# lordnn/OF_DIS

Measured on AMD Instinct MI355X. Metric: MPix/s (and frames/sec) 1080p op-point-2; avg EPE vs CPU ref, higher is better.
Workload: dtype f32; 1 GPU; run_OF_INT 1920x1080 op-point 2, 4096 pairs/GPU/step; width=1920, height=1080, channels=1, oppoint=2, batch_per_gpu=4096, streams=2, pairs_per_launch=2048, parallelism=frame-sharded x1

## Files before the change

### of_dis_amd/csrc/ofdis_internal.h

```cpp
#pragma once

#include <hip/hip_runtime.h>
#include <stdint.h>

namespace ofdis {

struct LevelGeom {
  int w, h;
  int pad;
  int W, H;
  int nopw, noph, npatch, offw, offh;
  float tmp_lb, tmp_ubw, tmp_ubh;
  int level;
};

struct PyrBaseArgs {
  const uint8_t *img_a, *img_b;
  int n, nf, W0, H0, noc;
  int padl, padt;
  int log2s;
  int w, h;
  float *out;
  int rgb_sad;
  int stereo;
};

struct PyrGradmagArgs {
  const uint8_t *img_a, *img_b;
  int n, nf, W0, H0, padl, padt, Wp, Hp;
  float *out;
  int stereo;
};

struct PyrDownArgs {
  const float *src;
  float *dst;
  int n2, w, h, noc;
};

struct PyrPadGradArgs {
  const float *lvl;
  float *img, *dx, *dy;
  int n2, w, h, noc, pad;
  int per_value;
};

struct PatchArgs {
  const float *img_a, *dx_a, *dy_a, *img_b;
  const float *prev;
  long prev_frame_stride;
  int prev_comp_stride, prev_elem_stride, prev_w;
  float *p_iter;
  float *pweight;
  int n, nop, noc, p, novals, steps;
  int costfct, patnorm, max_iter, min_iter;
  float dp_thresh_sq, dr_thresh, res_thresh, outlierthresh;
  float outlier_sq;
  int camlr;
  int wave_per_patch;
  int generic;
  int window;
  int quad;
  int x16;
  int absw;
  int aslots;
  int buf32;
  int fdiv;
  int maxres;
  int stage;
  LevelGeom g;
};

struct AggArgs {
  const float *p_iter, *pweight;
  const float *cg_p_iter, *cg_pweight;
  float *flow;
  int n, nop, noc, p, novals, steps;
  int absw;
  int aslots;
  int stage;
  LevelGeom g;
};

struct TvArgs {
  const float *img_a, *img_b;
  float *flow;
  float *wxs, *wys;
  float *du, *dv, *mask, *s;
  float *coef;
  float *t, *dt;
  float *Ix, *Iy, *Iz, *Ixx, *Ixy, *Iyy, *Ixz, *Iyz;
  long sp;
  int wrap;
  int skew_slots;
  int n, nop, noc, w, h, pad, W;
  float quarter_alpha, hdo3, hgo3, omega;
  int first_iter;
  int solverit;
  int camlr;
  int sor_generic;
  int sor_variant;
  int sor_point;
  int sor_cring;
  int sor_pack;
  int sor_rows2;
  int smsys;
  int prepd;
  int smsys2d;
  int smsys_prefetch;
  int smsys_small;
  int smsys_march;
  int smsys_deriv;
  int prepd_df;
  int sor_redblack;
  int lat;
};

struct UpArgs {
  const float *flow;
  float *out;
  int n, nop, wl, hl, log2s, W0, H0, offx, offy;
  int nt_store;
  int form;
  int f16, planar;
  float *out_r;
  int n_l;
};

struct LevelOutArgs {
  const float *flow;
  void *out;
  int n, nop, wl, hl, log2s;
  int f16, planar;
};

struct InitArgs {
  const float *init;
  float *out;
  int n, nop, W0, H0, padl, padt, log2k, wo, ho;
  float sc, scale;
};

struct FbArgs {
  const float *fw, *bw;
  uint8_t *occ_fw, *occ_bw;
  float *err_fw, *err_bw;
  int n, W, H;
  float alpha, beta;
};

struct FbLevelArgs {
  const float *gfw, *gbw;
  uint8_t *occ_fw, *occ_bw;
  float *err_fw, *err_bw;
  int n, W, H;
  float alpha, beta;
  int gw, gh, log2c, offx, offy;
};

struct LrArgs {
  const float *dl, *dr;
  uint8_t *occ_l, *occ_r;
  float *err_l, *err_r;
  int n, W, H;
  float alpha, beta;
};

struct WarpArgs {
  const uint8_t *img;
  const void *flow;
  void *out;
  uint8_t *valid;
  int n, W, H, noc;
  float scale;
  int out_f32;
  int f16, planar, level;
  int gw, gh, log2c, offx, offy;
};

constexpr int kInterpMaxT = 16;
struct InterpArgs {
  const uint8_t *img_a, *img_b;
  const void *flow_fw, *flow_bw;
  const uint8_t *occ_a, *occ_b;
  void *out;
  uint8_t *valid;
  int n, W, H, noc;
  int out_f32;
  int f16, planar, level;
  int gw, gh, log2c, offx, offy;
  int srows, scols;
  int nt;
  float t[kInterpMaxT];
};

void launch_warp(const WarpArgs &a, hipStream_t s);
// ... 32 lines not shown
```

### of_dis_amd/csrc/ofdis_kernels.hip

```cpp
#include "ofdis_internal.h"
#include "ofdis_math.h"

#include <algorithm>
#include <cstdlib>
#include <type_traits>
#include <utility>

#pragma clang fp contract(off)

namespace ofdis {
typedef float float4_u __attribute__((ext_vector_type(4), aligned(4)));
typedef float float4_v __attribute__((ext_vector_type(4)));

namespace {

#include "ofdis_tv_dev.inc"
#include "ofdis_agg_dev.inc"

inline unsigned ceil_div(long a, long b) { return (unsigned)((a + b - 1) / b); }

template <int V>
using Int = std::integral_constant<int, V>;
template <int... Vs, class F>
inline bool pick(int v, F &&f) {
// ... 98 lines not shown
          const uint4 v = reinterpret_cast<const uint4 *>(row)[q];
          s2 = __builtin_amdgcn_sad_u8(v.x, 0u, s2);
          s2 = __builtin_amdgcn_sad_u8(v.y, 0u, s2);
          s2 = __builtin_amdgcn_sad_u8(v.z, 0u, s2);
          s2 = __builtin_amdgcn_sad_u8(v.w, 0u, s2);
        }
      } else if (VB == 8) {
        const uint2 v = *reinterpret_cast<const uint2 *>(row);
        s2 = __builtin_amdgcn_sad_u8(v.x, 0u, s2);
        s2 = __builtin_amdgcn_sad_u8(v.y, 0u, s2);
      } else {
        s2 = __builtin_amdgcn_sad_u8(*reinterpret_cast<const unsigned *>(row), 0u, s2);
      }
      acc[by] = s2;
    }
#pragma unroll
    for (int by = 0; by < B; ++by) sum += acc[by];
  } else {
    for (int by = 0; by < B; ++by) {
      const int yy = clampi(y * B + by - a.padt, 0, a.H0 - 1);
      const uint8_t *row = src + (long)yy * a.W0;
      for (int bx = 0; bx < B; ++bx) {
        const int xc = clampi(x0 + bx, 0, a.W0 - 1);
        sum += row[ST && mir ? a.W0 - 1 - xc : xc];
      }
    }
  }
  a.out[t] = (float)sum * scale;
}

template <int L, bool ST = false>
__global__ __launch_bounds__(256) void k_pyr_base_rgb(PyrBaseArgs a) {
  constexpr int B = 1 << L, ND = 3 * B / 4;
  const long t = (long)blockIdx.x * 256 + threadIdx.x;
  if (t >= (long)a.nf * a.h * a.w) return;
  const int x = (int)(t % a.w);
  const long r = t / a.w;
  const int y = (int)(r % a.h), f = (int)(r / a.h);
  const long fs = (long)a.H0 * a.W0 * 3;
  bool mir;
  const uint8_t *src = pyr_src<ST>(a, f, fs, mir);
  const float scale = 1.0f / (float)(1 << (2 * L));
  const int x0 = x * B - a.padl;
  const int xs = ST && mir ? a.W0 - x0 - B : x0;
  unsigned sum[3] = {0u, 0u, 0u};
  if (x0 >= 0 && x0 + B <= a.W0 && (((uintptr_t)src + 3 * (long)xs) & 3) == 0 && ((3 * a.W0) & 3) == 0) {
    constexpr unsigned M[3][3] = {{0xFF0000FFu, 0x00FF0000u, 0x0000FF00u},
                                  {0x0000FF00u, 0xFF0000FFu, 0x00FF0000u},
                                  {0x00FF0000u, 0x0000FF00u, 0xFF0000FFu}};
    unsigned v[B][ND];
#pragma unroll
    for (int by = 0; by < B; ++by) {
      const int yy = clampi(y * B + by - a.padt, 0, a.H0 - 1);
      const unsigned *row = reinterpret_cast<const unsigned *>(src + ((long)yy * a.W0 + xs) * 3);
#pragma unroll
      for (int k = 0; k < ND; ++k) v[by][k] = row[k];
    }
#pragma unroll
    for (int by = 0; by < B; ++by)
#pragma unroll
      for (int k = 0; k < ND; ++k)
#pragma unroll
        for (int c = 0; c < 3; ++c) sum[c] = __builtin_amdgcn_sad_u8(v[by][k] & M[c][k % 3], 0u, sum[c]);
  } else {
    for (int c = 0; c < 3; ++c)
      for (int by = 0; by < B; ++by) {
        const int yy = clampi(y * B + by - a.padt, 0, a.H0 - 1);
        const uint8_t *row = src + (long)yy * a.W0 * 3 + c;
        for (int bx = 0; bx < B; ++bx) {
          const int xc = clampi(x0 + bx, 0, a.W0 - 1);
          sum[c] += row[(ST && mir ? a.W0 - 1 - xc : xc) * 3];
        }
      }
  }
#pragma unroll
  for (int c = 0; c < 3; ++c) a.out[t * 3 + c] = (float)sum[c] * scale;
}

__global__ __launch_bounds__(256) void k_pyr_down(PyrDownArgs a) {
  const int rw = a.w * a.noc;
  const long total = (long)a.n2 * a.h * rw;
  for (long t = (long)blockIdx.x * blockDim.x + threadIdx.x; t < total; t += (long)gridDim.x * blockDim.x) {
  const long r = t / rw;
  const int xc = (int)(t - r * rw), y = (int)(r % a.h), f = (int)(r / a.h);
  const int x = xc / a.noc, c = xc - x * a.noc;
  const long idx = (((long)f * a.h + y) * a.w + x) * a.noc + c;
  const int sw = 2 * a.w;
  const float *s = a.src + (long)f * (2 * a.h) * sw * a.noc;
  const float p = s[((2 * y) * sw + 2 * x) * a.noc + c], q = s[((2 * y) * sw + 2 * x + 1) * a.noc + c];
  const float u = s[((2 * y + 1) * sw + 2 * x) * a.noc + c], v = s[((2 * y + 1) * sw + 2 * x + 1) * a.noc + c];
  a.dst[idx] = ((p + q) + (u + v)) * 0.25f;
  }
}

__device__ __forceinline__ int reflect101(int i, int n) {
  if (n == 1) return 0;
  if (i < 0) return -i;
  if (i >= n) return 2 * n - 2 - i;
  return i;
}

template <bool ST = false>
__global__ __launch_bounds__(256) void k_pyr_gradmag(PyrGradmagArgs a) {
  const int X = blockIdx.x * blockDim.x + threadIdx.x, Y = blockIdx.y, f = blockIdx.z;
  if (X >= a.Wp) return;
  const long fs = (long)a.H0 * a.W0;
  bool mir = false;
  const uint8_t *src;
  if constexpr (ST) {
    const int q = f / a.n, i = f - q * a.n;
    mir = (q & 1) != 0;
    src = (q == 0 || q == 3 ? a.img_a : a.img_b) + (long)i * fs;
  } else {
    src = f < a.n ? a.img_a + (long)f * fs : a.img_b + (long)(f - a.n) * fs;
  }
  const int xm = reflect101(X - 1, a.Wp), xp = reflect101(X + 1, a.Wp);
  const int ym = reflect101(Y - 1, a.Hp), yp = reflect101(Y + 1, a.Hp);
  auto px = [&](int xx, int yy) {
    const int xc = clampi(xx - a.padl, 0, a.W0 - 1);
    return (float)src[(long)clampi(yy - a.padt, 0, a.H0 - 1) * a.W0 + (ST && mir ? a.W0 - 1 - xc : xc)];
  };
  const float tm = px(xp, ym) - px(xm, ym);
  const float t0 = px(xp, Y) - px(xm, Y);
  const float tp = px(xp, yp) - px(xm, yp);
  const float sm = (px(xm, ym) + px(xp, ym)) * 0.125f + px(X, ym) * 0.25f;
  const float sp = (px(xm, yp) + px(xp, yp)) * 0.125f + px(X, yp) * 0.25f;
  const float dx = (tm + tp) * 0.125f + t0 * 0.25f, dy = sp - sm;
  a.out[((long)f * a.Hp + Y) * a.Wp + X] = sqrtf(dx * dx + dy * dy);
}

__global__ __launch_bounds__(256) void k_pyr_pad_grad(PyrPadGradArgs a) {
  const int W = a.w + 2 * a.pad, H = a.h + 2 * a.pad;
  const long total = (long)a.n2 * H * W;
  for (long t = (long)blockIdx.x * blockDim.x + threadIdx.x; t < total; t += (long)gridDim.x * blockDim.x) {
  const long r = t / W;
  const int X = (int)(t - r * W), Y = (int)(r % H), f = (int)(r / H);
  const long idx = ((long)f * H + Y) * W + X;
  const int sx = X - a.pad, sy = Y - a.pad;
  const int noc = a.noc, w = a.w;
  const float *L = a.lvl + (long)f * a.h * a.w * noc;
  const bool inside = sx >= 0 && sx < a.w && sy >= 0 && sy < a.h;
  for (int c = 0; c < noc; ++c) {
    const long o = idx * noc + c;
    if (inside) {
      const int xm = reflect101(sx - 1, a.w), xp = reflect101(sx + 1, a.w);
      const int ym = reflect101(sy - 1, a.h), yp = reflect101(sy + 1, a.h);
#define PX(xx, yy) L[((yy) * w + (xx)) * noc + c]
      const float tm = PX(xp, ym) - PX(xm, ym);
      const float t0 = PX(xp, sy) - PX(xm, sy);
      const float tp = PX(xp, yp) - PX(xm, yp);
      const float sm = (PX(xm, ym) + PX(xp, ym)) * 0.125f + PX(sx, ym) * 0.25f;
      const float sp = (PX(xm, yp) + PX(xp, yp)) * 0.125f + PX(sx, yp) * 0.25f;
      a.img[o] = PX(sx, sy);
      a.dx[o] = (tm + tp) * 0.125f + t0 * 0.25f;
      a.dy[o] = sp - sm;
#undef PX
    } else {
      a.img[o] = L[(clampi(sy, 0, a.h - 1) * w + clampi(sx, 0, a.w - 1)) * noc + c];
      a.dx[o] = 0.0f;
      a.dy[o] = 0.0f;
    }
  }
  }
}

template <int NOC>
__global__ __launch_bounds__(256) void k_pyr_pad_grad_v(PyrPadGradArgs a) {
  const int W = a.w + 2 * a.pad, H = a.h + 2 * a.pad, RW = W * NOC;
  const long total = (long)a.n2 * H * RW;
  for (long t = (long)blockIdx.x * blockDim.x + threadIdx.x; t < total; t += (long)gridDim.x * blockDim.x) {
    const long r = t / RW;
    const int xc = (int)(t - r * RW), Y = (int)(r % H), f = (int)(r / H);
    const int X = xc / NOC, c = xc - X * NOC;
    const int sx = X - a.pad, sy = Y - a.pad;
    const int w = a.w;
    const float *L = a.lvl + (long)f * a.h * a.w * NOC;
    if (sx >= 0 && sx < a.w && sy >= 0 && sy < a.h) {
      const int xm = reflect101(sx - 1, a.w), xp = reflect101(sx + 1, a.w);
      const int ym = reflect101(sy - 1, a.h), yp = reflect101(sy + 1, a.h);
#define PX(xx, yy) L[((yy) * w + (xx)) * NOC + c]
      const float tm = PX(xp, ym) - PX(xm, ym);
      const float t0 = PX(xp, sy) - PX(xm, sy);
      const float tp = PX(xp, yp) - PX(xm, yp);
      const float sm = (PX(xm, ym) + PX(xp, ym)) * 0.125f + PX(sx, ym) * 0.25f;
      const float sp = (PX(xm, yp) + PX(xp, yp)) * 0.125f + PX(sx, yp) * 0.25f;
      a.img[t] = PX(sx, sy);
      a.dx[t] = (tm + tp) * 0.125f + t0 * 0.25f;
      a.dy[t] = sp - sm;
#undef PX
    } else {
      a.img[t] = L[(clampi(sy, 0, a.h - 1) * w + clampi(sx, 0, a.w - 1)) * NOC + c];
      a.dx[t] = 0.0f;
      a.dy[t] = 0.0f;
    }
  }
}

}
void launch_pyr_base(const PyrBaseArgs &a, hipStream_t s) {
  const unsigned blocks = ceil_div((long)a.nf * a.h * a.w, 256);
  if (a.stereo) {
    if (a.noc == 1 && pick<2, 3, 4, 5>(a.log2s, [&](auto L) { k_pyr_base_gray<L, true><<<blocks, 256, 0, s>>>(a); })) return;
    if (a.noc == 3 && a.rgb_sad && pick<2, 3, 4>(a.log2s, [&](auto L) { k_pyr_base_rgb<L, true><<<blocks, 256, 0, s>>>(a); }))
      return;
    k_pyr_base<true><<<dim3(ceil_div(a.w, 256), a.h, a.nf), 256, 0, s>>>(a);
    return;
  }
  if (a.noc == 1 && pick<2, 3, 4, 5>(a.log2s, [&](auto L) { k_pyr_base_gray<L><<<blocks, 256, 0, s>>>(a); })) return;
  if (a.noc == 3 && a.rgb_sad && pick<2, 3, 4>(a.log2s, [&](auto L) { k_pyr_base_rgb<L><<<blocks, 256, 0, s>>>(a); }))
    return;
  k_pyr_base<<<dim3(ceil_div(a.w, 256), a.h, a.nf), 256, 0, s>>>(a);
}
void launch_pyr_gradmag(const PyrGradmagArgs &a, hipStream_t s) {
  if (a.stereo) k_pyr_gradmag<true><<<dim3(ceil_div(a.Wp, 256), a.Hp, a.nf), 256, 0, s>>>(a);
  else k_pyr_gradmag<<<dim3(ceil_div(a.Wp, 256), a.Hp, a.nf), 256, 0, s>>>(a);
}
void launch_pyr_down(const PyrDownArgs &a, hipStream_t s) {
  k_pyr_down<<<std::min(ceil_div((long)a.n2 * a.h * a.w * a.noc, 256), 1u << 22), 256, 0, s>>>(a);
}
void launch_pyr_pad_grad(const PyrPadGradArgs &a, hipStream_t s) {
  const long px = (long)a.n2 * (a.h + 2 * a.pad) * (a.w + 2 * a.pad);
  if (a.noc == 3 && a.per_value) k_pyr_pad_grad_v<3><<<std::min(ceil_div(px * 3, 256), 1u << 22), 256, 0, s>>>(a);
  else k_pyr_pad_grad<<<std::min(ceil_div(px, 256), 1u << 22), 256, 0, s>>>(a);
}
namespace {


constexpr int kPatchWaves = 4;

template <int N>
__device__ __forceinline__ float row_shl(float v) {
  return __builtin_bit_cast(float, __builtin_amdgcn_update_dpp(0, __builtin_bit_cast(int, v), 0x100 + N, 0xF, 0xF, false));
}

template <int R, int JM>
__device__ __forceinline__ void eigen_reduce(const float *lds, int rs, int n, int lane, float (&out)[R]) {
  __builtin_amdgcn_fence(__ATOMIC_RELEASE, "wavefront");
  __builtin_amdgcn_wave_barrier();
  __builtin_amdgcn_fence(__ATOMIC_ACQUIRE, "wavefront");
  const int r = lane >> 3, s = lane & 7;
  const int pairs = n >> 3;
  const bool odd = ((n >> 2) & 1) != 0;
  float acc = 0.0f, first = 0.0f, tail = 0.0f;
  if (r < R) {
    if (JM == 1) {
      const float4 A = *reinterpret_cast<const float4 *>(lds + r * 64 + s * 8);
      const float4 B = *reinterpret_cast<const float4 *>(lds + r * 64 + s * 8 + 4);
      const float e[8] = {A.x, A.y, A.z, A.w, B.x, B.y, B.z, B.w};
      first = e[0];
      acc = first;
#pragma unroll
      for (int c = 1; c < 8; ++c)
        if (c < pairs) acc = acc + e[c];
#pragma unroll
      for (int c = 0; c < 8; ++c)
        if (c == pairs) tail = e[c];
    } else {
      const float *x = lds + r * rs;
      first = x[s];
      acc = first;
      for (int c = 1; c < pairs; ++c) acc = acc + x[s + 8 * c];
      tail = x[pairs * 8 + s];
    }
  }
  float rl = pairs > 0 ? acc + row_shl<4>(acc) : first;
  if (odd && pairs > 0) rl = rl + tail;
  const float t = rl + row_shl<2>(rl);
  const float tot = t + row_shl<1>(t);
#pragma unroll
  for (int k = 0; k < R; ++k)
    out[k] = __builtin_bit_cast(float, __builtin_amdgcn_readlane(__builtin_bit_cast(int, tot), k * 8));
  __builtin_amdgcn_wave_barrier();
}

template <int JM>
__device__ __forceinline__ void lds_store(float *lds, int n, int lane, const float (&v)[JM]) {
  if (JM == 1) {
    lds[(lane & 7) * 8 + (lane >> 3)] = lane < n ? v[0] : 0.0f;
    return;
  }
#pragma unroll
  for (int j = 0; j < JM; ++j) {
    const int e = lane + 64 * j;
    if (e < n) lds[e] = v[j];
  }
}

struct Llt2 {
  float L00, L10, L11;
};
__device__ __forceinline__ Llt2 llt2_factor(float H00, float H01, float H11) {
  Llt2 f{H00, H01, H11};
  if (!(H00 <= 0.0f)) {
    f.L00 = sqrtf(H00);
    f.L10 = H01 / f.L00;
    const float t = H11 - f.L10 * f.L10;
    if (!(t <= 0.0f)) f.L11 = sqrtf(t);
  }
  return f;
}
__device__ __forceinline__ void llt2_solve(const Llt2 &f, float b0, float b1, float &x0, float &x1) {
  const float y0 = b0 / f.L00;
  const float y1 = (b1 - f.L10 * y0) / f.L11;
  x1 = y1 / f.L11;
  x0 = (y0 - f.L10 * x1) / f.L00;
}
__device__ __forceinline__ float llt1_factor(float H) { return !(H <= 0.0f) ? sqrtf(H) : H; }
__device__ __forceinline__ float llt1_solve(float L, float b) {
  const float y = b / L;
  return y / L;
}

struct LltRcp {
  float r00, r11;
  bool ok;
};
__device__ __forceinline__ bool mdiv_in(float a) { return fabsf(a) >= 0x1p-60f && fabsf(a) <= 0x1p60f; }
__device__ __forceinline__ bool mdiv_pivot(float L) { return fabsf(L) >= 0x1p-30f && fabsf(L) <= 0x1p30f; }
__device__ __forceinline__ float mdiv(float a, float L, float y) {
  const float q0 = a * y;
  const float r = __builtin_fmaf(-q0, L, a);
  return __builtin_fmaf(r, y, q0);
}
template <int NOP>
__device__ __forceinline__ LltRcp llt_rcp(const Llt2 &f, float L1, bool enable) {
  LltRcp r;
  if (NOP == 2) {
    r.r00 = 1.0f / f.L00;
    r.r11 = 1.0f / f.L11;
    r.ok = enable && mdiv_pivot(f.L00) && mdiv_pivot(f.L11);
  } else {
    r.r00 = 1.0f / L1;
    r.r11 = 0.0f;
    r.ok = enable && mdiv_pivot(L1);
  }
  return r;
}
__device__ __forceinline__ void llt2_solve_fast(const Llt2 &f, const LltRcp &rc, float b0, float b1, float &x0,
                                                float &x1) {
  const float y0 = mdiv(b0, f.L00, rc.r00);
  const float n1 = b1 - f.L10 * y0;
  const float y1 = mdiv(n1, f.L11, rc.r11);
  x1 = mdiv(y1, f.L11, rc.r11);
  const float n3 = y0 - f.L10 * x1;
  x0 = mdiv(n3, f.L00, rc.r00);
  const bool slow = !(rc.ok && mdiv_in(b0) && mdiv_in(n1) && mdiv_in(y1) && mdiv_in(n3));
  if (__builtin_amdgcn_ballot_w64(slow) != 0 && slow) llt2_solve(f, b0, b1, x0, x1);
}
__device__ __forceinline__ float llt1_solve_fast(float L, const LltRcp &rc, float b) {
  const float y = mdiv(b, L, rc.r00);
  float x = mdiv(y, L, rc.r00);
  const bool slow = !(rc.ok && mdiv_in(b) && mdiv_in(y));
  if (__builtin_amdgcn_ballot_w64(slow) != 0 && slow) x = llt1_solve(L, b);
  return x;
}


__device__ __forceinline__ void patch_decode(const PatchArgs &a, long gq, int &f, int &pxi, int &pyi, float &ptr0,
                                             float &ptr1) {
  const LevelGeom &g = a.g;
  f = (int)(gq / g.npatch);
  const int ip = (int)(gq % g.npatch);
  pxi = ip / g.noph;
  pyi = ip % g.noph;
  ptr0 = (float)(pxi * a.steps + g.offw);
  ptr1 = (float)(pyi * a.steps + g.offh);
}
template <int NOP>
__device__ __forceinline__ void hessian_regularise(float &H00, float H01, float &H11) {
  if (NOP == 2) {
    if (H00 * H11 - H01 * H01 == 0.0f) {
      H00 = (float)((double)H00 + 1e-10);
      H11 = (float)((double)H11 + 1e-10);
    }
  } else if (H00 == 0.0f) {
    H00 = (float)((double)H00 + 1e-10);
// ... 5325 lines not shown
```

### of_dis_amd/csrc/ofdis_runtime.cpp

```cpp
#include <hip/hip_runtime.h>

#include <algorithm>
#include <chrono>
#include <cmath>
#include <cstdio>
#include <cstdlib>
#include <cstring>
#include <functional>
#include <map>
#include <mutex>
#include <string>
#include <vector>

#include "../../include/ofdis.h"
#include "ofdis_internal.h"

using namespace ofdis;

namespace {

const char *const kKernelNames[] = {"pyr_base", "pyr_down", "pyr_pad_grad", "patch",    "aggregate", "tv_prep",
                                    "tv_deriv", "tv_system", "tv_sor",       "tv_final", "upsample",  "tv_level",
                                    "fb_check", "fb_check_err",
                                    "upsample_f16", "upsample_planar", "upsample_planar_f16", "level_out",
// ... 469 lines not shown
      tv.img_a = dir == 0 ? img : img + bd * fsp;
      tv.img_b = dir == 0 ? img + bd * fsp : img;
      tv.flow = dir == 0 ? flow : flow_bw;
      tv.du = t0;
      tv.dv = t0 + pl;
      tv.mask = t0 + 2 * pl;
      tv.coef = t0 + 3 * pl;
      tv.s = t0 + 11 * pl;
      tv.wxs = t0 + 12 * pl;
      tv.wys = t0 + 13 * pl;
      tv.sp = sp;
      tv.wrap = g.h <= g.w;
      tv.skew_slots = tv.wrap ? g.w * g.h : (g.w + g.h - 1) * g.h;
      float *cp = t0 + 14 * pl;
      const size_t cpl = pl * noc;
      tv.t = cp;
      tv.dt = cp + cpl;
      tv.Iz = tv.dt;
      tv.Ix = cp + 2 * cpl;
      tv.Iy = cp + 3 * cpl;
      tv.Ixx = cp + 4 * cpl;
      tv.Ixy = cp + 5 * cpl;
      tv.Iyy = cp + 6 * cpl;
      tv.Ixz = cp + 7 * cpl;
      tv.Iyz = cp + 8 * cpl;
      tv.n = n;
      tv.nop = nop;
      tv.noc = noc;
      tv.w = g.w;
      tv.h = g.h;
      tv.pad = g.pad;
      tv.W = g.W;
      tv.quarter_alpha = 0.25f * p->tv_alpha;
      tv.hgo3 = p->tv_gamma * 0.5f / 3.0f;
      tv.hdo3 = p->tv_delta * 0.5f / 3.0f;
      tv.omega = p->tv_sor;
      tv.solverit = p->tv_solverit;
      tv.camlr = dir;
      tv.sor_generic = c->opt_sor_generic;
      tv.sor_variant = c->opt_sor_pipe;
      tv.sor_cring = c->opt_sor_cring;
      tv.sor_pack = c->opt_sor_pack;      tv.sor_rows2 = c->opt_sor_rows2;
      tv.smsys = c->opt_smsys;
      tv.smsys2d = c->opt_smsys2d == 2 ? c->call_frames < 512 : c->opt_smsys2d;
      tv.smsys_march = c->opt_smsys_march;
      tv.smsys_prefetch = c->opt_smsys_prefetch;
      tv.smsys_small = c->opt_smsys_small;
      tv.smsys_deriv = c->opt_smsys_deriv;
      tv.prepd_df = c->opt_prepd_df;
      tv.sor_redblack = c->opt_sor_mode == 1;
      tv.sor_point = p->omp_build && nop == 2;
      tv.prepd = c->opt_prepd;
      return tv;
    };
    if (times) HIP_OK(hipEventRecord(ev[3], s));
    timed(c, 4, s, [&] { launch_aggregate(ag, s); });
    const bool bw_level = bw && (sl > p->sc_l || P.bidir);
    if (bw_level) {
      AggArgs ab = ag;
      ab.p_iter = pb.p_iter;
      ab.pweight = pb.pweight;
      ab.cg_p_iter = P.fb ? pa.p_iter : nullptr;
      ab.cg_pweight = P.fb ? pa.pweight : nullptr;
      ab.absw = absw_bw;
      ab.flow = flow_bw;
      timed(c, 4, s, [&] { launch_aggregate(ab, s); });
    }
    if (times) HIP_OK(hipEventRecord(ev[4], s));
    int rc = capture(c, s, c->cap_dis, sl, P, flow);
    if (rc) return rc;

    for (int dir = 0; dir < (bw_level ? 2 : 1) && p->usetvref && n_inner > 0; ++dir) {
      TvArgs tv = make_tv(dir);
      tv.lat = tv_level_rb_ok(tv);
      tv.smsys_deriv = !tv.lat && tv_deriv_fused(tv);
      if (tv_prepd_ok(tv)) {
        timed(c, 5, s, [&] { launch_tv_prepd(tv, s); });
      } else {
        timed(c, 5, s, [&] { launch_tv_prep(tv, s); });
        timed(c, 6, s, [&] {
          launch_tv_deriv1(tv, s);
          launch_tv_deriv2(tv, s);
        });
      }
      if (tv.lat) {
        timed(c, 11, s, [&] { launch_tv_level_rb(tv, n_inner, s); });
        continue;
      }
      for (int it = 0; it < n_inner; ++it) {
        tv.first_iter = it == 0;
        timed(c, 7, s, [&] {
          if (tv_smsys_ok(tv)) {
            launch_tv_smsys(tv, s);
          } else {
            launch_tv_smooth(tv, s);
            launch_tv_system(tv, s);
          }
        });
        timed(c, 8, s, [&] { launch_tv_sor(tv, s); });
      }
      timed(c, 9, s, [&] { launch_tv_final(tv, s); });
    }
    if (times) {
      HIP_OK(hipEventRecord(ev[5], s));
      HIP_OK(hipEventSynchronize(ev[5]));
      StageTimes st;
      float t01, t12, t23, t34, t45;
      hipEventElapsedTime(&t01, ev[0], ev[1]);
      hipEventElapsedTime(&t12, ev[1], ev[2]);
      hipEventElapsedTime(&t23, ev[2], ev[3]);
      hipEventElapsedTime(&t34, ev[3], ev[4]);
      hipEventElapsedTime(&t45, ev[4], ev[5]);
      st.pconst = t01;
      st.pinit = std::max(0.0, (double)t12 - t01);
      st.poptim = std::max(0.0, (double)t23 - t12);
      st.cflow = t34;
      st.tvopt = t45;
      times->push_back(st);
    }
    rc = capture(c, s, c->cap_tv, sl, P, flow);
    if (rc) return rc;
  }
  if (times)
    for (auto &e : ev) hipEventDestroy(e);
  return hipGetLastError() == hipSuccess ? OFDIS_OK : OFDIS_ERR_DEVICE;
}

void print_times(const Plan &P, const std::vector<StageTimes> &t, double total_ms, int verbosity) {
  if (verbosity > 1) {
    for (size_t k = 0; k < t.size(); ++k) {
      const int sl = P.sc_f - (int)k;
      const LevelGeom &g = P.lv[sl - P.sc_l];
      const double all = t[k].pconst + t[k].pinit + t[k].poptim + t[k].cflow + t[k].tvopt;
      std::printf("TIME (Sc: %i, #p:%6i, pconst, pinit, poptim, cflow, tvopt, total): %8.2f %8.2f %8.2f %8.2f %8.2f -> %8.2f ms.\n",
                  sl, g.npatch, t[k].pconst, t[k].pinit, t[k].poptim, t[k].cflow, t[k].tvopt, all);
    }
  }
  if (verbosity > 0) std::printf("TIME (O.Flow Run-Time   ) (ms): %3g\n", total_ms);
}

int check_device(int device) {
  int count = 0;
  if (hipGetDeviceCount(&count) != hipSuccess || count <= 0) return OFDIS_ERR_NO_DEVICE;
  if (device < 0 || device >= count) return OFDIS_ERR_INVALID_ARGUMENT;
  hipDeviceProp_t prop;
  if (hipGetDeviceProperties(&prop, device) != hipSuccess) return OFDIS_ERR_DEVICE;
  if (std::strncmp(prop.gcnArchName, "gfx950", 6) != 0) {
    std::fprintf(stderr, "ofdis: device %d is %s, this build targets gfx950 only\n", device, prop.gcnArchName);
    return OFDIS_ERR_NO_DEVICE;
  }
  return OFDIS_OK;
}

int run_pyramid(ofdis_context *c, char *ws, const Plan &P, const uint8_t *a, const uint8_t *b, hipStream_t s) {
  const int n2 = P.nfr, na = P.seq ? P.nfr : P.stereo ? P.n / 2 : P.n;
  if (P.gradmag) {
    float *lvl0 = (float *)(ws + P.off_lvl[0]);
    float *bufA = (float *)(ws + P.off_gm), *bufB = bufA + (size_t)n2 * P.Wp * P.Hp;
    PyrGradmagArgs g{};
    g.img_a = a;
    g.img_b = b;
    g.n = na;
    g.nf = n2;
    g.W0 = P.W0;
    g.H0 = P.H0;
    g.padl = P.padl;
    g.padt = P.padt;
    g.Wp = P.Wp;
    g.Hp = P.Hp;
    g.stereo = P.stereo;
    g.out = P.sc_l == 0 ? lvl0 : bufA;
    timed(c, 0, s, [&] { launch_pyr_gradmag(g, s); });
    const float *src = bufA;
    int w = P.Wp, h = P.Hp;
    for (int l = 1; l <= P.sc_l; ++l) {
      PyrDownArgs pd{};
      pd.src = src;
      pd.dst = l == P.sc_l ? lvl0 : ((l & 1) ? bufB : bufA);
      pd.n2 = n2;
      pd.w = w /= 2;
      pd.h = h /= 2;
      pd.noc = 1;
      timed(c, 1, s, [&] { launch_pyr_down(pd, s); });
      src = pd.dst;
    }
  } else {
    PyrBaseArgs pb{};
    pb.img_a = a;
    pb.img_b = b;
    pb.n = na;
    pb.nf = n2;
    pb.W0 = P.W0;
    pb.H0 = P.H0;
    pb.noc = P.noc;
    pb.padl = P.padl;
    pb.padt = P.padt;
    pb.log2s = P.sc_l;
    pb.w = P.lv[0].w;
    pb.h = P.lv[0].h;
    pb.out = (float *)(ws + P.off_lvl[0]);
    pb.rgb_sad = c->opt_pyr_rgb;
    pb.stereo = P.stereo;
    timed(c, 0, s, [&] { launch_pyr_base(pb, s); });
  }
  for (size_t i = 1; i < P.lv.size(); ++i) {
    PyrDownArgs pd{};
    pd.src = (const float *)(ws + P.off_lvl[i - 1]);
    pd.dst = (float *)(ws + P.off_lvl[i]);
    pd.n2 = n2;
    pd.w = P.lv[i].w;
    pd.h = P.lv[i].h;
    pd.noc = P.noc;
    timed(c, 1, s, [&] { launch_pyr_down(pd, s); });
  }
  for (size_t i = 0; i < P.lv.size(); ++i) {
    PyrPadGradArgs pg{};
    pg.lvl = (const float *)(ws + P.off_lvl[i]);
    pg.img = (float *)(ws + P.off_img[i]);
    pg.dx = (float *)(ws + P.off_dx[i]);
    pg.dy = (float *)(ws + P.off_dy[i]);
    pg.n2 = n2;
    pg.w = P.lv[i].w;
    pg.h = P.lv[i].h;
    pg.noc = P.noc;
    pg.pad = P.pad;
    pg.per_value = c->opt_pad_grad_v;
    timed(c, 2, s, [&] { launch_pyr_pad_grad(pg, s); });
  }
  return hipGetLastError() == hipSuccess ? OFDIS_OK : OFDIS_ERR_DEVICE;
}

Plan batch_plan(const ofdis_params *p, int n, int width, int height, bool init = false, int bidir = 0,
                int stride = 0, int stereo = 0) {
  const int d = 1 << (p->sc_f + (init ? 1 : 0));
  const int padw = (width % d) ? d - width % d : 0, padh = (height % d) ? d - height % d : 0;
  Plan P = make_plan(p, stereo ? 2 * n : n, width + padw, height + padh, p->p_samp_s, init, bidir != 0, stride);
  P.stereo = stereo != 0;
  P.off_up_bw = P.total;
  if (bidir == 2 || stereo == 2) P.total = align_up(P.total + sizeof(float) * (size_t)n * width * height * P.nop);
  if (bidir == 3) P.total = align_up(P.total + 2 * (size_t)n * width * height);
  P.W0 = width;
  P.H0 = height;
  P.padw = padw;
  P.padh = padh;
  P.padl = padw / 2;
  P.padt = padh / 2;
  return P;
}

}

extern "C" {

int ofdis_context_create(int device, ofdis_context **out) {
  if (!out) return OFDIS_ERR_INVALID_ARGUMENT;
  *out = nullptr;
  int rc = check_device(device);
  if (rc) return rc;
  HIP_OK(hipSetDevice(device));
  ofdis_context *c = new ofdis_context();
  c->device = device;
  if (hipStreamCreateWithFlags(&c->stream, hipStreamNonBlocking) != hipSuccess) {
    delete c;
    return OFDIS_ERR_DEVICE;
  }
  warm_kernels_module(c->stream);
  warm_tvrb_module(c->stream);
  if (hipStreamSynchronize(c->stream) != hipSuccess) {
    hipStreamDestroy(c->stream);
    delete c;
    return OFDIS_ERR_DEVICE;
  }
  *out = c;
  return OFDIS_OK;
}

void ofdis_context_destroy(ofdis_context *c) {
  if (!c) return;
  hipSetDevice(c->device);
  if (c->gexec) {
    hipDeviceSynchronize();
    hipGraphExecDestroy(c->gexec);
    c->gexec = nullptr;
  }
  if (c->ws_pending) hipEventSynchronize(c->ev_ws);
  if (c->stream) hipStreamSynchronize(c->stream);
  drain_timing(c);
  for (auto e : c->pool) hipEventDestroy(e);
  if (c->ws) hipFree(c->ws);
  if (c->warp_buf) hipFree(c->warp_buf);
  for (auto &L : c->lanes) {
    if (L.s) hipStreamSynchronize(L.s);
    if (L.ws) hipFree(L.ws);
    if (L.done) hipEventDestroy(L.done);
    if (L.s) hipStreamDestroy(L.s);
  }
  if (c->entry) hipEventDestroy(c->entry);
  if (c->ev_null) hipEventDestroy(c->ev_null);
  if (c->ev_ws) hipEventDestroy(c->ev_ws);
  if (c->stream) hipStreamDestroy(c->stream);
  delete c;
}

namespace {

int run_upsample(ofdis_context *c, char *ws, const Plan &P, const ofdis_params *p, void *flow_out, hipStream_t s,
                 bool backward = false, const OutFmt &fmt = OutFmt(), float *disp_r = nullptr) {
  if (fmt.level) {
    LevelOutArgs lo{};
    lo.flow = (const float *)(ws + P.off_flow[0]);
    lo.out = flow_out;
    lo.n = P.n;
    lo.nop = P.nop;
    lo.wl = P.lv[0].w;
    lo.hl = P.lv[0].h;
    lo.log2s = p->sc_l;
    lo.f16 = fmt.f16;
    lo.planar = fmt.planar;
    timed(c, 17, s, [&] { launch_level_out(lo, s); });
    return hipGetLastError() == hipSuccess ? OFDIS_OK : OFDIS_ERR_DEVICE;
  }
  UpArgs up{};
  up.flow = (const float *)(ws + (backward ? P.off_flow_bw[0] : P.off_flow[0]));
  up.out = (float *)flow_out;
  up.n = P.n;
  up.nop = P.nop;
  up.wl = P.lv[0].w;
  up.hl = P.lv[0].h;
  up.log2s = p->sc_l;
  up.W0 = P.W0;
  up.H0 = P.H0;
  up.offx = P.padl;
  up.offy = P.padt;
  up.nt_store = c->opt_nt_store;
  up.form = c->opt_up_form == 3 ? (P.W0 >= 1024 && (c->call_lanes >= 2 || c->call_frames < 1024) ? 1 : 0)
                                 : c->opt_up_form;
  up.f16 = fmt.f16;
  up.planar = fmt.planar;
  up.out_r = disp_r;
  up.n_l = disp_r ? P.n / 2 : P.n;
  timed(c, fmt.f16 ? (fmt.planar ? 16 : 14) : fmt.planar ? 15 : 10, s, [&] { launch_upsample(up, s); });
  return hipGetLastError() == hipSuccess ? OFDIS_OK : OFDIS_ERR_DEVICE;
}

int run_init(ofdis_context *c, char *ws, const Plan &P, const ofdis_params *p, const float *init, hipStream_t s) {
  InitArgs ia{};
  ia.init = init;
  ia.out = (float *)(ws + P.off_init);
  ia.n = P.n;
  ia.nop = P.nop;
  ia.W0 = P.W0;
  ia.H0 = P.H0;
  ia.padl = P.padl;
  ia.padt = P.padt;
  ia.log2k = p->sc_f + 1;
  ia.wo = P.Wp >> (p->sc_f + 1);
  ia.ho = P.Hp >> (p->sc_f + 1);
  ia.sc = (float)std::pow(2.0, -p->sc_f - 1);
  ia.scale = 1.f / (float)(1 << (2 * (p->sc_f + 1)));
  launch_init_area(ia, s);
  return hipGetLastError() == hipSuccess ? OFDIS_OK : OFDIS_ERR_DEVICE;
}

struct BidirOut {
  float *flow_bw = nullptr;
  uint8_t *occ_fw = nullptr, *occ_bw = nullptr;
  float *err_fw = nullptr, *err_bw = nullptr;
  float alpha = 0.f, beta = 0.f;
  bool stereo = false;
  bool checks() const { return occ_fw || occ_bw || err_fw || err_bw; }
  BidirOut at(size_t f0, size_t px) const {
    BidirOut o = *this;
    if (flow_bw) o.flow_bw += f0 * px * (stereo ? 1 : 2);
    if (occ_fw) o.occ_fw += f0 * px;
    if (occ_bw) o.occ_bw += f0 * px;
    if (err_fw) o.err_fw += f0 * px;
    if (err_bw) o.err_bw += f0 * px;
    return o;
// ... 1538 lines not shown
```

Measured before the change: 330,700 MPix/s.

## Skip gradients for target frames and add LDS-tiled pad-grad kernel

Adds an ngrad bound so x/y gradients are written only for frames that need them. For plain forward pairs that means the reference frames, since the target frames never use gradients. It also adds a new single-channel pad/gradient kernel that stages a source tile plus halo in shared memory and computes padded image and Sobel gradients from it, so overlapping neighbour reads no longer go to global memory. The tiled path only runs when per_value is set, and gradient skipping depends on the plan-shape heuristic correctly identifying forward-pair layouts.

```diff
diff --git a/of_dis_amd/csrc/ofdis_internal.h b/of_dis_amd/csrc/ofdis_internal.h
--- a/of_dis_amd/csrc/ofdis_internal.h
+++ b/of_dis_amd/csrc/ofdis_internal.h
@@ -42,6 +42,7 @@
   const float *lvl;
   float *img, *dx, *dy;
   int n2, w, h, noc, pad;
+  int ngrad;
   int per_value;
 };
 
diff --git a/of_dis_amd/csrc/ofdis_kernels.hip b/of_dis_amd/csrc/ofdis_kernels.hip
--- a/of_dis_amd/csrc/ofdis_kernels.hip
+++ b/of_dis_amd/csrc/ofdis_kernels.hip
@@ -274,15 +274,77 @@
       const float sm = (PX(xm, ym) + PX(xp, ym)) * 0.125f + PX(sx, ym) * 0.25f;
       const float sp = (PX(xm, yp) + PX(xp, yp)) * 0.125f + PX(sx, yp) * 0.25f;
       a.img[o] = PX(sx, sy);
-      a.dx[o] = (tm + tp) * 0.125f + t0 * 0.25f;
-      a.dy[o] = sp - sm;
+      if (f < a.ngrad) {
+        a.dx[o] = (tm + tp) * 0.125f + t0 * 0.25f;
+        a.dy[o] = sp - sm;
+      }
 #undef PX
     } else {
       a.img[o] = L[(clampi(sy, 0, a.h - 1) * w + clampi(sx, 0, a.w - 1)) * noc + c];
-      a.dx[o] = 0.0f;
-      a.dy[o] = 0.0f;
-    }
-  }
+      if (f < a.ngrad) {
+        a.dx[o] = 0.0f;
+        a.dy[o] = 0.0f;
+      }
+    }
+  }
+  }
+}
+
+constexpr int kPgTileW = 256;
+constexpr int kPgWholeW = 320;
+constexpr int kPgRows = 16;
+__global__ __launch_bounds__(256) void k_pyr_pad_grad_s(PyrPadGradArgs a, int tw, int rows) {
+  extern __shared__ float pg_st[];
+  const int W = a.w + 2 * a.pad, H = a.h + 2 * a.pad;
+  const int X0 = blockIdx.z * tw, Y0 = blockIdx.y * rows, f = blockIdx.x;
+  const int nx = min(tw, W - X0), ny = min(rows, H - Y0);
+  if (nx <= 0 || ny <= 0) return;
+  const int cx0 = max(clampi(X0 - a.pad, 0, a.w - 1) - 1, 0), cx1 = min(clampi(X0 + nx - 1 - a.pad, 0, a.w - 1) + 1, a.w - 1);
+  const int ry0 = max(clampi(Y0 - a.pad, 0, a.h - 1) - 1, 0), ry1 = min(clampi(Y0 + ny - 1 - a.pad, 0, a.h - 1) + 1, a.h - 1);
+  const int nc = cx1 - cx0 + 1, nr = ry1 - ry0 + 1;
+  const float *L = a.lvl + (size_t)f * ((size_t)a.h * a.w) + ((size_t)ry0 * a.w + cx0);
+  {
+    int c = threadIdx.x, r = 0;
+    while (c >= nc) { c -= nc; ++r; }
+    for (int i = threadIdx.x; i < nr * nc; i += 256) {
+      pg_st[i] = L[r * a.w + c];
+      c += 256;
+      while (c >= nc) { c -= nc; ++r; }
+    }
+  }
+  __syncthreads();
+  const bool grad = f < a.ngrad;
+  const size_t o0 = ((size_t)f * H + Y0) * W + X0;
+  float *img = a.img + o0, *dx = a.dx + o0, *dy = a.dy + o0;
+  int xl = threadIdx.x, yl = 0;
+  while (xl >= nx) { xl -= nx; ++yl; }
+  for (int i = threadIdx.x; i < ny * nx; i += 256) {
+    const int sx = X0 + xl - a.pad, sy = Y0 + yl - a.pad;
+    const int o = yl * W + xl;
+#define PX(xx, yy) pg_st[((yy) - ry0) * nc + ((xx) - cx0)]
+    if (sx >= 0 && sx < a.w && sy >= 0 && sy < a.h) {
+      img[o] = PX(sx, sy);
+      if (grad) {
+        const int xm = reflect101(sx - 1, a.w), xp = reflect101(sx + 1, a.w);
+        const int ym = reflect101(sy - 1, a.h), yp = reflect101(sy + 1, a.h);
+        const float tm = PX(xp, ym) - PX(xm, ym);
+        const float t0 = PX(xp, sy) - PX(xm, sy);
+        const float tp = PX(xp, yp) - PX(xm, yp);
+        const float sm = (PX(xm, ym) + PX(xp, ym)) * 0.125f + PX(sx, ym) * 0.25f;
+        const float sp = (PX(xm, yp) + PX(xp, yp)) * 0.125f + PX(sx, yp) * 0.25f;
+        dx[o] = (tm + tp) * 0.125f + t0 * 0.25f;
+        dy[o] = sp - sm;
+      }
+    } else {
+      img[o] = PX(clampi(sx, 0, a.w - 1), clampi(sy, 0, a.h - 1));
+      if (grad) {
+        dx[o] = 0.0f;
+        dy[o] = 0.0f;
+      }
+    }
+#undef PX
+    xl += 256;
+    while (xl >= nx) { xl -= nx; ++yl; }
   }
 }
 
@@ -307,13 +369,17 @@
       const float sm = (PX(xm, ym) + PX(xp, ym)) * 0.125f + PX(sx, ym) * 0.25f;
       const float sp = (PX(xm, yp) + PX(xp, yp)) * 0.125f + PX(sx, yp) * 0.25f;
       a.img[t] = PX(sx, sy);
-      a.dx[t] = (tm + tp) * 0.125f + t0 * 0.25f;
-      a.dy[t] = sp - sm;
+      if (f < a.ngrad) {
+        a.dx[t] = (tm + tp) * 0.125f + t0 * 0.25f;
+        a.dy[t] = sp - sm;
+      }
 #undef PX
     } else {
       a.img[t] = L[(clampi(sy, 0, a.h - 1) * w + clampi(sx, 0, a.w - 1)) * NOC + c];
-      a.dx[t] = 0.0f;
-      a.dy[t] = 0.0f;
+      if (f < a.ngrad) {
+        a.dx[t] = 0.0f;
+        a.dy[t] = 0.0f;
+      }
     }
   }
 }
@@ -343,7 +409,13 @@
 void launch_pyr_pad_grad(const PyrPadGradArgs &a, hipStream_t s) {
   const long px = (long)a.n2 * (a.h + 2 * a.pad) * (a.w + 2 * a.pad);
   if (a.noc == 3 && a.per_value) k_pyr_pad_grad_v<3><<<std::min(ceil_div(px * 3, 256), 1u << 22), 256, 0, s>>>(a);
-  else k_pyr_pad_grad<<<std::min(ceil_div(px, 256), 1u << 22), 256, 0, s>>>(a);
+  else if (a.noc == 1 && a.per_value) {
+    const int W = a.w + 2 * a.pad, H = a.h + 2 * a.pad;
+    const int tiles = W <= kPgWholeW ? 1 : (int)ceil_div(W, kPgTileW), groups = (int)ceil_div(H, kPgRows);
+    const int tw = (int)ceil_div(W, tiles), rows = (int)ceil_div(H, groups);
+    const size_t lds = sizeof(float) * std::min(rows + 2, a.h) * std::min(tw + 2, a.w);
+    k_pyr_pad_grad_s<<<dim3(a.n2, groups, tiles), 256, lds, s>>>(a, tw, rows);
+  } else k_pyr_pad_grad<<<std::min(ceil_div(px, 256), 1u << 22), 256, 0, s>>>(a);
 }
 namespace {
 
diff --git a/of_dis_amd/csrc/ofdis_runtime.cpp b/of_dis_amd/csrc/ofdis_runtime.cpp
--- a/of_dis_amd/csrc/ofdis_runtime.cpp
+++ b/of_dis_amd/csrc/ofdis_runtime.cpp
@@ -645,6 +645,11 @@
   return OFDIS_OK;
 }
 
+int grad_frames(const Plan &P) {
+  const bool forward_pairs = !P.fb && !P.bidir && !P.seq && !P.stereo && !P.gradmag && P.nfr == 2 * P.n && P.bdist == P.n;
+  return forward_pairs ? P.n : P.nfr;
+}
+
 int run_pyramid(ofdis_context *c, char *ws, const Plan &P, const uint8_t *a, const uint8_t *b, hipStream_t s) {
   const int n2 = P.nfr, na = P.seq ? P.nfr : P.stereo ? P.n / 2 : P.n;
   if (P.gradmag) {
@@ -717,6 +722,7 @@
     pg.h = P.lv[i].h;
     pg.noc = P.noc;
     pg.pad = P.pad;
+    pg.ngrad = grad_frames(P);
     pg.per_value = c->opt_pad_grad_v;
     timed(c, 2, s, [&] { launch_pyr_pad_grad(pg, s); });
   }
```

New measurement: 334,100 MPix/s (median of 6 runs). 1.01x the previous value.
